# AlexanderRipar/Octree_Ray_Tracing

Measured on AMD Instinct MI355X. Metric: Mrays/sec primary traversal (depth-12 SVO-DAG, raygen+trace+shade per frame), higher is better.
Workload: dtype f32

## Files before the change

### include/och_gpu.h

```cpp
#ifndef OCH_GPU_H
#define OCH_GPU_H

#include <stddef.h>
#include <stdint.h>

#ifdef __cplusplus
extern "C" {
#endif

#define OCH_GPU_ABI_VERSION 1
#define OCH_MAX_VIEWS 8

#if defined(__GNUC__)
#define OCH_API __attribute__((visibility("default")))
#else
#define OCH_API
#endif

typedef enum och_status {
    OCH_OK = 0,
    OCH_E_INVALID = -1,
    OCH_E_HIP = -2,
    OCH_E_NODEV = -3,
    OCH_E_RCP_MODEL = -4,
// ... 17 lines not shown

typedef struct och_camera {
    float pos[3];
    float rot[9];
    float fov_factor;
    float aspect;
    float view_x;
    float view_y;
    int32_t width, height;
} och_camera;

typedef struct och_pool_info {
    uint64_t device_bytes;
    uint32_t n_nodes;
    uint32_t root;
    int32_t depth;
    int32_t index_base;
    float miss_t;
    int32_t rcp_log2_entries;
    int32_t device;
} och_pool_info;

OCH_API int och_abi_version(void);
OCH_API const char *och_last_error(void);
OCH_API int och_discarded_error(int *hip_error, int *count, char *what, size_t what_cap, int reset);
OCH_API int och_device_count(int *count);
OCH_API int och_device_list(int *devices, int capacity, int *count);

OCH_API int och_host_rcp_lut(uint32_t *lut, int *log2_entries);
OCH_API uint32_t och_rcp_from_lut(uint32_t xbits, const uint32_t *lut, int log2_entries);
OCH_API int och_rcp_lut_error(const uint32_t *lut, int log2_entries, double *max_rel_error);

OCH_API int och_gpu_pool_create(const uint32_t *nodes, uint32_t n_nodes, uint32_t root, int depth,
                                int index_base, float miss_t, int device, och_gpu_pool **out);
OCH_API int och_gpu_pool_destroy(och_gpu_pool *pool);
OCH_API int och_gpu_pool_info(const och_gpu_pool *pool, och_pool_info *info);
OCH_API int och_gpu_pool_update(och_gpu_pool *pool, uint32_t first, uint32_t count,
                                const uint32_t *nodes, uint32_t root);
OCH_API int och_gpu_set_rcp_lut(och_gpu_pool *pool, const uint32_t *lut, int log2_entries);
OCH_API int och_gpu_set_palette(och_gpu_pool *pool, const uint32_t *rgba, uint32_t n_voxels);
OCH_API int och_gpu_set_stream(och_gpu_pool *pool, void *hip_stream);
OCH_API int och_gpu_synchronize(och_gpu_pool *pool);
typedef enum och_option {
    OCH_OPT_BLOCK = 1,
    OCH_OPT_LAYOUT = 4,
    OCH_OPT_TILE_ORDER = 5,
    OCH_OPT_BOUNCE_COMPACT = 6,
    OCH_OPT_CULL = 8,
    OCH_OPT_TIMING = 10,
    OCH_OPT_PLAN = 11,
    OCH_OPT_SPLIT = 14,
    OCH_OPT_SPLIT_SEGS = 15,
    OCH_OPT_SPLIT_LEVEL = 16,
    OCH_OPT_SPLIT_TILES = 17
} och_option;
OCH_API int och_gpu_set_option(och_gpu_pool *pool, int option, int value);
OCH_API int och_gpu_get_option(const och_gpu_pool *pool, int option, int *value);
OCH_API int och_gpu_set_stamp_buffer(och_gpu_pool *pool, uint64_t *stamps, uint32_t capacity_waves);
OCH_API int och_gpu_occupancy(const och_gpu_pool *pool, int kind, int *blocks_per_cu);
OCH_API int och_gpu_last_kernel_ms(och_gpu_pool *pool, float *ms);
OCH_API int och_gpu_set_launch_events(och_gpu_pool *pool, void *start_event, void *stop_event);

OCH_API int och_gpu_trace(och_gpu_pool *pool, float ox, float oy, float oz, float dx, float dy, float dz,
                          int32_t *hit_direction, uint32_t *hit_voxel, float *hit_time);
OCH_API int och_gpu_trace_batch(och_gpu_pool *pool, const float *origin, int origin_stride,
                                const float *dirs, uint32_t n,
                                int32_t *hit_direction, uint32_t *hit_voxel, float *hit_time);
OCH_API int och_gpu_trace_batch_dev(och_gpu_pool *pool, const float *origin, int origin_stride,
                                    const float *dirs, uint32_t n,
                                    int32_t *hit_direction, uint32_t *hit_voxel, float *hit_time,
                                    uint32_t *push_count);

OCH_API int och_gpu_trace_batch_tiled_dev(och_gpu_pool *pool, const float *origin, int origin_stride,
                                          const float *dirs, uint32_t n, uint32_t width,
                                          int32_t *hit_direction, uint32_t *hit_voxel, float *hit_time,
                                          uint32_t *push_count);
OCH_API int och_gpu_trace_batch_image(och_gpu_pool *pool, const float *origin, int origin_stride,
                                      const float *dirs, uint32_t n, uint32_t width,
                                      int32_t *hit_direction, uint32_t *hit_voxel, float *hit_time);
OCH_API int och_gpu_plan_batch_tiled(och_gpu_pool *pool, const float *origin, int origin_stride,
                                     const float *dirs, uint32_t n, uint32_t width);

OCH_API int och_gpu_trace_bounce_batch_dev(och_gpu_pool *pool, const float *origin, int origin_stride,
                                           const float *dirs, uint32_t n,
                                           int32_t *hit_direction, uint32_t *hit_voxel, float *hit_time,
                                           int32_t *bounce_direction, uint32_t *bounce_voxel, float *bounce_time,
                                           uint32_t *push_count);

OCH_API int och_camera_setup(float px, float py, float pz, float yaw, float pitch, float fov,
                             int width, int height, och_camera *cam);
OCH_API int och_gpu_raygen_dev(och_gpu_pool *pool, const och_camera *cam, float *dirs);
OCH_API int och_gpu_render(och_gpu_pool *pool, const och_camera *cam, uint32_t *rgba);
OCH_API int och_gpu_render_dev(och_gpu_pool *pool, const och_camera *cam, uint32_t *rgba_slice,
                               int row_chunk, int shard, int n_shards);
OCH_API int och_shard_rows(int height, int row_chunk, int n_shards);
OCH_API int och_gpu_render_views_dev(och_gpu_pool *pool, const och_camera *cams, int n_views, uint32_t *rgba_slices,
                                     int row_chunk, int shard, int n_shards);
OCH_API int och_gpu_plan_views(och_gpu_pool *pool, const och_camera *cams, int n_views, int row_chunk, int shard,
                               int n_shards);
OCH_API int och_gpu_render_bounce_views_dev(och_gpu_pool *pool, const och_camera *cams, int n_views,
                                            uint32_t *rgba_slices, int row_chunk, int shard, int n_shards);
OCH_API int och_gpu_render_ssaa_views_dev(och_gpu_pool *pool, const och_camera *cams, int n_views, int s,
                                          uint32_t *rgba, size_t capacity_pixels);
OCH_API int och_gpu_render_ssaa(och_gpu_pool *pool, const och_camera *cam, int s, uint32_t *rgba,
                                size_t capacity_pixels);
enum { OCH_LIGHT_SUN = 1, OCH_LIGHT_AO = 2 };
typedef struct och_light {
// ... 228 lines not shown
```

### octree_ray_tracing_amd/csrc/och_internal.h

```cpp
#pragma once
#include <hip/hip_runtime.h>
#include <stdint.h>

#include <vector>

#include "../../include/och_gpu.h"
#include "och_tiles.h"

namespace och {

struct DevPool {
    const uint32_t *nodes;
    uint32_t n_slots;
    const uint32_t *lut;
    uint32_t rcp_xlo;
    uint32_t rcp_xspan;
    uint32_t root;
    int32_t packed;
    int32_t depth;
    int32_t lut_shift;
    uint32_t miss_bits;
    float half_voxel;
    uint32_t dim_lo;
    uint32_t dim_span;
    int32_t cull;
    float cull_lo[3], cull_hi[3];
    int32_t cam_cull;
};

constexpr double kCameraCullRcpError = 0x1p-10;

bool occupied_box(const uint32_t *nodes, uint32_t n_nodes, uint32_t root, int depth, int base, int32_t lo[3],
                  int32_t hi[3]);

int report(int status, const char *msg);

void clear_pending_error(const char *launcher);
struct EntryScope {
    const char *prev;
    explicit EntryScope(const char *name);
    ~EntryScope();
};
#define OCH_ENTRY() const och::EntryScope och_entry_scope_(__func__)

int pool_drain(och_gpu_pool *pool);
int pool_write_slots(och_gpu_pool *pool, uint32_t first, uint32_t count, const uint32_t *raw,
                     const uint32_t *packed, bool full);
int pool_commit(och_gpu_pool *pool, uint32_t root, uint32_t packed_root, bool packed, uint64_t writer,
                const int32_t *box_lo, const int32_t *box_hi);
int pool_mark_torn(och_gpu_pool *pool);
int pool_scatter_slots(och_gpu_pool *pool, const uint32_t *ids, uint32_t count, const uint32_t *raw,
                       const uint32_t *packed);
hipError_t launch_scatter_slots(const uint32_t *ids, const uint32_t *raw, const uint32_t *packed, uint32_t count,
                                uint32_t *d_raw, uint32_t *d_packed, hipStream_t stream);
uint64_t pool_serial(const och_gpu_pool *pool);
void *pool_stream(const och_gpu_pool *pool);
int pool_palette_size(const och_gpu_pool *pool, int *n_voxels);
uint64_t pool_last_writer(const och_gpu_pool *pool);

int comm_ranks(const och_comm *comm, int *n_ranks, int *rank, int *device);
int comm_all_gather(och_comm *comm, const void *send, void *recv, size_t bytes, hipStream_t stream);
int comm_gather(och_comm *comm, const void *send, void *recv, size_t bytes, int root, hipStream_t stream);
void comm_abort(och_comm *comm);

struct DevFrame {
    och_camera cams[OCH_MAX_VIEWS];
    int32_t n_views;
    const uint32_t *palette;
    uint32_t n_voxels;
    uint32_t *out;
    uint8_t *codes;
    int32_t row_chunk, shard, n_shards, slice_rows;
    const int32_t *chunk_map;
};

constexpr int kBounceBlock = 256;

struct Schedule {
    int block;
    int tile_order;
// ... 50 lines not shown
```

### octree_ray_tracing_amd/csrc/och_kernels.hip

```cpp
#include <hip/hip_ext.h>
#include <hip/hip_runtime.h>
#include <stdint.h>

#include <type_traits>

#include "och_internal.h"

#define OCH_LAUNCH_TIMED(sc, kernel, grid, block, lds, stream, ...)                                                   \
    do {                                                                                                             \
        clear_pending_error(__func__);                                                                               \
        if ((sc).ev_start || (sc).ev_stop)                                                                           \
            hipExtLaunchKernelGGL(kernel, grid, block, (uint32_t)(lds), stream, (sc).ev_start, (sc).ev_stop, 0u,     \
                                  __VA_ARGS__);                                                                      \
        else                                                                                                         \
            hipLaunchKernelGGL(kernel, grid, block, lds, stream, __VA_ARGS__);                                       \
    } while (0)

namespace och {
namespace {

constexpr uint32_t kX86DefaultNaN = 0xFFC00000u;

constexpr int kMaxViews = OCH_MAX_VIEWS;

// ... 492 lines not shown

struct FastDiv {
    uint32_t d, m, s;
    __host__ void init(uint32_t divisor)
    {
        d = divisor ? divisor : 1u;
        divisor = d;
        s = 0;
        while ((1ull << s) < divisor) ++s;
        m = (uint32_t)((((1ull << s) - divisor) << 32) / divisor + 1);
    }
    __device__ __forceinline__ uint32_t div(uint32_t n) const
    {
        return (uint32_t)(((uint64_t)__umulhi(n, m) + n) >> s);
    }
};

struct TiledArraySource {
    static constexpr bool kProvenMiss = false;
    static constexpr bool kTileTable = false;
    const float *origin;
    const float *dirs;
    int origin_stride;
    uint32_t n, width, tiles_x, tiles;
    FastDiv by_tiles_x;
    __host__ __device__ __forceinline__ uint32_t count() const { return tiles * 64u; }
    __device__ __forceinline__ bool at(uint32_t tile, uint32_t lane, float *o, float *d, uint32_t &out) const
    {
        const uint32_t ty = by_tiles_x.div(tile), tx = tile - ty * tiles_x;
        const uint32_t col = tx * 8u + (lane & 7u), row = ty * 8u + (lane >> 3);
        if (col >= width) return false;
        const uint32_t i = row * width + col;
        if (i >= n) return false;
        const float *po = origin + (size_t)origin_stride * i;
        const float *pd = dirs + 3 * (size_t)i;
        o[0] = po[0]; o[1] = po[1]; o[2] = po[2];
        d[0] = pd[0]; d[1] = pd[1]; d[2] = pd[2];
        out = i;
        return true;
    }
    __device__ __forceinline__ bool get_wave_culled(uint32_t wave_base, uint32_t lane, const DevPool &, bool,
                                                    float *o, float *d, uint32_t &out, bool &miss) const
    {
        miss = false;
        return at(__builtin_amdgcn_readfirstlane(wave_base >> 6), lane, o, d, out);
    }
};

struct CameraSource {
    static constexpr bool kProvenMiss = true;
    static constexpr bool kTileTable = true;
    och_camera cam[kMaxViews];
    CameraView view[kMaxViews];
    int32_t row_chunk, shard, n_shards, slice_rows, width, height;
    uint32_t slice_pixels, n_tiles;
    const uint2 *tiles;
    FastDiv by_row_chunk;
    const int32_t *chunk_map;
    __device__ __forceinline__ int global_row(int chunk, int within) const
    {
        const int g = chunk_map ? chunk_map[chunk] : chunk * n_shards + shard;
        return g < 0 ? height : g * row_chunk + within;
    }
    __host__ __device__ __forceinline__ uint32_t count() const { return n_tiles * 64u; }
    __device__ __forceinline__ bool get_wave_culled(uint32_t wave_base, uint32_t lane, const DevPool &P, bool cull,
                                                    float *o, float *d, uint32_t &out, bool &miss) const
    {
        return get_tile_culled(tile(wave_base), lane, P, cull, o, d, out, miss);
    }
    __device__ __forceinline__ bool get_tile_culled(uint2 e, uint32_t lane, const DevPool &P, bool cull, float *o, float *d,
                                                    uint32_t &out, bool &miss) const
    {
        uint32_t view;
        int col, srow, row;
        miss = false;
        if (!locate(e, lane, view, col, srow, row)) return false;
        const och_camera &C = cam[view];
        out = view * slice_pixels + (uint32_t)srow * (uint32_t)width + (uint32_t)col;
        float ru, rv, rw;
        camera_rot(C, col, row, ru, rv, rw);
        if (cull && P.cam_cull && camera_proven_miss(this->view[view], ru, rv, rw)) {
            miss = true;
            return true;
        }
        o[0] = C.pos[0]; o[1] = C.pos[1]; o[2] = C.pos[2];
        camera_ray_from(ru, rv, rw, d);
        return true;
    }
    __device__ __forceinline__ uint2 tile(uint32_t wave_base) const
    {
#if defined(__HIP_DEVICE_COMPILE__)
        typedef const __attribute__((address_space(4))) uint32_t *table_ptr;
#else
        typedef const uint32_t *table_ptr;
#endif
        const table_ptr w = (table_ptr)(uintptr_t)tiles + 2u * __builtin_amdgcn_readfirstlane(wave_base >> 6);
        const uint2 e = make_uint2(w[0], w[1]);
        return make_uint2(__builtin_amdgcn_readfirstlane(e.x), __builtin_amdgcn_readfirstlane(e.y));
    }
    __device__ __forceinline__ uint32_t sample_word(uint32_t wave_base, uint32_t lane, int log2_s) const
    {
        const uint2 e = tile(wave_base);
        const uint32_t w = (uint32_t)width >> log2_s, h = (uint32_t)height >> log2_s;
        const uint32_t x = (e.x & 0xFFFFu) + lane % kTileW, y = (e.y >> 16) + lane / kTileW;
        return (((e.x >> 16) & 15u) * h + (y >> log2_s)) * w + (x >> log2_s);
    }
    __device__ __forceinline__ bool locate(uint2 e, uint32_t lane, uint32_t &view, int &col, int &srow, int &row) const
    {
        if (e.x & kTileEmpty) return false;
        view = (e.x >> 16) & 15u;
        col = (int)((e.x & 0xFFFFu) + lane % kTileW);
        srow = (int)((e.y >> 16) + lane / kTileW);
        row = (int)((e.y & 0xFFFFu) + lane / kTileW);
        if (e.x & kTileInside) return true;
        if (col >= width || srow >= slice_rows) return false;
        if (e.x & kTileRows) {
            const int chunk = (int)by_row_chunk.div((uint32_t)srow);
            row = global_row(chunk, srow - chunk * row_chunk);
        }
        return row < height;
    }
};


template <bool kCount>
struct HitSink {
    int32_t *dir;
    uint32_t *voxel;
    uint32_t *t;
    uint32_t *push;
    __device__ __forceinline__ void put(uint32_t i, const Hit &h) const
    {
        dir[i] = h.dir;
        voxel[i] = h.voxel;
// ... 151 lines not shown
    if (key != ~0u) atomicMin(&lds_stack[best0 + pix], (key << 6) | lane);
    __syncthreads();
    if (valid) {
        const uint32_t b = lds_stack[best0 + pix];
        if (b == ~0u ? seg == 0u : (b & 63u) == lane) K.put(out, h);
    }
}

template <class Src, class Sink, int kPacked, bool kCount, bool kSplit, bool kDiag>
__global__ __attribute__((amdgpu_num_sgpr(80))) void k_trace_grid(DevPool P, Src S, Sink K, const uint32_t *__restrict__ order,
                             uint32_t *__restrict__ cost, uint64_t *stamps, uint32_t stamp_cap,
                             const uint32_t *__restrict__ split_tasks, uint32_t split_level)
{
    extern __shared__ uint32_t lds_stack[];
    if constexpr (!kDiag) {
        cost = nullptr;
        stamps = nullptr;
    }
    const uint64_t t0 = stamps ? realtime() : 0;
    const uint64_t c0 = cost ? __builtin_amdgcn_s_memtime() : 0;
    uint32_t blk = blockIdx.x;
    if constexpr (!Src::kTileTable) blk = order ? order[blockIdx.x] : blockIdx.x;
    const uint32_t lane = threadIdx.x & 63u;
    const uint32_t wave_base = kSplit ? blk * 64u : blk * blockDim.x + (threadIdx.x & ~63u);
    float o[3], d[3];
    uint32_t out;
    bool miss, have;
    if constexpr (Src::kTileTable) {
        const uint2 ent = S.tile(wave_base);
        if constexpr (kSplit) {
            if (ent.x >> 31) {
                split_tile<Src, Sink, kPacked>(P, S, K, ent, split_tasks, split_level, lds_stack);
                if (stamps) stamp(stamps, stamp_cap, t0, 64);
                return;
            }
        }
        have = S.get_tile_culled(ent, lane, P, kCount ? P.cull == 2 : P.cull != 0, o, d, out, miss);
    } else {
        have = wave_base + lane < S.count() &&
               S.get_wave_culled(wave_base, lane, P, kCount ? P.cull == 2 : P.cull != 0, o, d, out, miss);
    }
    if (have) {
        if (miss) {
            K.put(out, Hit{OCH_EXIT, 0u, P.miss_bits, 0u});
        } else {
            Ray r;
            ray_trace<kPacked, kCount, true, kAsmLoad>(r, P, o, d, stack_column(lds_stack, P.depth), blockDim.x,
                                                      !(Src::kProvenMiss && P.cam_cull));
            K.put(out, ray_result<kPacked, kAsmLoad>(r, P));
        }
    }
    if (cost && threadIdx.x == 0) cost[blk] = (uint32_t)(__builtin_amdgcn_s_memtime() - c0);
    if (stamps) stamp(stamps, stamp_cap, t0, 64);
}

template <uint32_t kBit>
__device__ __forceinline__ uint32_t lane_xor(uint32_t v)
{
    if constexpr (kBit == 1u)
        return (uint32_t)__builtin_amdgcn_update_dpp(0, (int)v, 0xB1, 0xF, 0xF, true);
    else if constexpr (kBit == 2u)
        return (uint32_t)__builtin_amdgcn_update_dpp(0, (int)v, 0x4E, 0xF, 0xF, true);
    else if constexpr (kBit == 8u)
        return (uint32_t)__builtin_amdgcn_update_dpp(0, (int)v, 0x128, 0xF, 0xF, true);
    else if constexpr (kBit == 4u || kBit == 16u)
        return (uint32_t)__builtin_amdgcn_ds_swizzle((int)v, (int)(0x1Fu | (kBit << 10)));
    else {
        static_assert(kBit == 32u, "a lane bit");
        return __builtin_amdgcn_permlane32_swap(v, v, false, false)[1];
    }
}

template <int kLog2S>
__device__ __forceinline__ uint32_t block_sum(uint32_t v)
{
    v += lane_xor<1u>(v);
    v += lane_xor<8u>(v);
    if constexpr (kLog2S >= 2) {
        v += lane_xor<2u>(v);
        v += lane_xor<16u>(v);
    }
    if constexpr (kLog2S >= 3) {
        v += lane_xor<4u>(v);
        v += lane_xor<32u>(v);
    }
    return v;
}

template <int kLog2S>
__device__ __forceinline__ void ssaa_resolve(uint32_t *out, uint32_t word, uint32_t lane, uint32_t colour)
{
    constexpr uint32_t kS = 1u << kLog2S;
    const uint32_t rb = block_sum<kLog2S>(colour & 0x00FF00FFu), ga = block_sum<kLog2S>((colour >> 8) & 0x00FF00FFu);
    if (word != ~0u && (lane & (kS - 1u)) == 0 && ((lane >> 3) & (kS - 1u)) == 0) {
        constexpr uint32_t half = (kS * kS / 2u) * 0x00010001u;
        out[word] = (((rb + half) >> (2 * kLog2S)) & 0x00FF00FFu) | ((((ga + half) >> (2 * kLog2S)) & 0x00FF00FFu) << 8);
    }
}

template <int kPacked, int kLog2S>
__global__ __attribute__((amdgpu_num_sgpr(80))) void k_trace_ssaa(DevPool P, CameraSource S, FrameSink K, uint64_t *stamps,
                                                                  uint32_t stamp_cap)
{
    extern __shared__ uint32_t lds_stack[];
    const uint64_t t0 = stamps ? realtime() : 0;
    const uint32_t blk = blockIdx.x;
// ... 450 lines not shown
                                                            int row_chunk, int n_shards, int slice_rows, int n_views,
                                                            const int32_t *__restrict__ owner, int sun_shade, int ao_shade)
{
    __shared__ uint32_t lut[256];
    lut[threadIdx.x] = table[threadIdx.x];
    __syncthreads();
    const int col = (blockIdx.x * 256 + threadIdx.x) * 4;
    const int row = blockIdx.y, view = blockIdx.z;
    if (col >= width || row >= height) return;
    const size_t src = gathered_row(row, row_chunk, n_shards, slice_rows, n_views, view, owner) * width + col;
    typedef uint32_t u32x2 __attribute__((ext_vector_type(2)));
    typedef uint32_t u32x4 __attribute__((ext_vector_type(4)));
    const u32x2 c = __builtin_nontemporal_load(reinterpret_cast<const u32x2 *>(gathered + src));
    const u32x4 px = {lit_code_word(lut, c.x & 0xFFFFu, sun_shade, ao_shade), lit_code_word(lut, c.x >> 16, sun_shade, ao_shade),
                      lit_code_word(lut, c.y & 0xFFFFu, sun_shade, ao_shade), lit_code_word(lut, c.y >> 16, sun_shade, ao_shade)};
    __builtin_nontemporal_store(px, reinterpret_cast<u32x4 *>(frames + ((size_t)view * height + row) * width + col));
}

__global__ __launch_bounds__(256) void k_scatter_slots(const uint32_t *__restrict__ ids,
                                                       const uint32_t *__restrict__ raw,
                                                       const uint32_t *__restrict__ packed, uint32_t count,
                                                       uint32_t *__restrict__ d_raw, uint32_t *__restrict__ d_packed)
{
    const uint32_t i = blockIdx.x * 256u + threadIdx.x;
    if (i >= count * 8u) return;
    const uint32_t slot = ids[i >> 3], w = i & 7u;
    d_raw[(size_t)slot * 8 + w] = raw[i];
    if (packed) d_packed[(size_t)slot * 8 + w] = packed[i];
}

constexpr size_t kStaticLds = 64;
size_t stack_bytes(int depth, int block)
{
    const size_t e = (size_t)(depth + 1) * block, c = (e + 2) / 3;
    return 4 * (c > kStaticLds ? c : kStaticLds) + 4 * e;
}

bool tiles_fit(const Schedule &sc, int block)
{
    return sc.tiles && block > 0 && sc.tiles_block == (uint32_t)block &&
           (uint64_t)sc.tiles_grid * ((uint32_t)block / 64u) <= sc.tiles_n;
}

template <class Src, class Sink, int kPacked, bool kCount>
hipError_t launch_as(const DevPool &p, const Src &s, const Sink &k, uint32_t n, const Schedule &sc, hipStream_t stream)
{
    if (!Src::kTileTable && n == 0) return hipSuccess;
    const int block = sc.block;
    const size_t lds = stack_bytes(p.depth, block);
    const uint32_t grid = (n + (uint32_t)block - 1) / (uint32_t)block;
    if constexpr (Src::kTileTable) {
        if (!tiles_fit(sc, block)) return hipErrorInvalidValue;
        const bool diag = sc.cost || sc.stamps;
        if (sc.split_tasks) {
            if constexpr (kPacked && !kCount) {
                if (block != 64) return hipErrorInvalidValue;
                if (diag)
                    OCH_LAUNCH_TIMED(sc, (k_trace_grid<Src, Sink, kPacked, kCount, true, true>), dim3(sc.tiles_grid),
                                     dim3(block), lds, stream, p, s, k, nullptr, sc.cost, sc.stamps, sc.stamp_cap,
                                     sc.split_tasks, sc.split_level);
                else
                    OCH_LAUNCH_TIMED(sc, (k_trace_grid<Src, Sink, kPacked, kCount, true, false>), dim3(sc.tiles_grid),
                                     dim3(block), lds, stream, p, s, k, nullptr, nullptr, nullptr, 0u, sc.split_tasks,
                                     sc.split_level);
                return hipGetLastError();
            }
            return hipErrorInvalidValue;
        }
        if (diag)
            OCH_LAUNCH_TIMED(sc, (k_trace_grid<Src, Sink, kPacked, kCount, false, true>), dim3(sc.tiles_grid), dim3(block),
                             lds, stream, p, s, k, nullptr, sc.cost, sc.stamps, sc.stamp_cap, nullptr, 0u);
        else
            OCH_LAUNCH_TIMED(sc, (k_trace_grid<Src, Sink, kPacked, kCount, false, false>), dim3(sc.tiles_grid), dim3(block),
                             lds, stream, p, s, k, nullptr, nullptr, nullptr, 0u, nullptr, 0u);
        return hipGetLastError();
    }
    OCH_LAUNCH_TIMED(sc, (k_trace_grid<Src, Sink, kPacked, kCount, false, true>), dim3(grid), dim3(block), lds, stream, p, s,
                     k, sc.order_n == grid ? sc.order : nullptr, sc.cost, sc.stamps, sc.stamp_cap, nullptr,
                     0u);
    return hipGetLastError();
}

template <class Src, class Sink, bool kCount>
hipError_t launch(const DevPool &p, const Src &s, const Sink &k, uint32_t n, const Schedule &sc, hipStream_t stream)
{
    return p.packed ? launch_as<Src, Sink, 1, kCount>(p, s, k, n, sc, stream)
                    : launch_as<Src, Sink, 0, kCount>(p, s, k, n, sc, stream);
}

template <class Src, class Sink, bool kCount>
hipError_t launch_bounce(const DevPool &p, const Src &s, const Sink &k, uint32_t n, const Schedule &sc, hipStream_t stream)
{
    if (!Src::kTileTable && n == 0) return hipSuccess;
    const int block = sc.block > kBounceBlock ? sc.block : kBounceBlock;
    const size_t queue = 8u * (size_t)block * sizeof(uint32_t);
    const size_t lds = stack_bytes(p.depth, block) > queue ? stack_bytes(p.depth, block) : queue;
    dim3 grid((n + block - 1) / block);
    const uint32_t *order = sc.order_n == grid.x ? sc.order : nullptr;
    if constexpr (Src::kTileTable) {
        if (!tiles_fit(sc, block) || sc.split_tasks) return hipErrorInvalidValue;
        grid.x = sc.tiles_grid;
        order = nullptr;
    }
    if (p.packed)
        OCH_LAUNCH_TIMED(sc, (k_trace_bounce<Src, Sink, 1, kCount>), grid, dim3(block), lds, stream, p, s, k,
                         sc.bounce_compact, order, sc.cost, sc.stamps, sc.stamp_cap);
    else
        OCH_LAUNCH_TIMED(sc, (k_trace_bounce<Src, Sink, 0, kCount>), grid, dim3(block), lds, stream, p, s, k,
                         sc.bounce_compact, order, sc.cost, sc.stamps, sc.stamp_cap);
    return hipGetLastError();
}

CameraSource camera_source(const DevPool &p, const DevFrame &f, const Schedule &sc)
{
    CameraSource src;
    for (int v = 0; v < f.n_views; ++v) {
        src.cam[v] = f.cams[v];
        CameraView &V = src.view[v];
        V.pos_ok = 1;
        for (int a = 0; a < 3; ++a) {
            const float o = f.cams[v].pos[a];
            const float lo = p.cull_lo[a] - 0x1p-16F, hi = p.cull_hi[a] + 0x1p-16F;
            V.lo[a] = lo - o;
            V.hi[a] = hi - o;
            V.pos_ok &= (o > 1.0F && o < 2.0F) ? 1 : 0;
        }
    }
    src.row_chunk = f.row_chunk;
    src.shard = f.shard;
    src.n_shards = f.n_shards;
    src.slice_rows = f.slice_rows;
    src.width = f.cams[0].width;
    src.height = f.cams[0].height;
    src.slice_pixels = (uint32_t)f.slice_rows * (uint32_t)src.width;
    src.by_row_chunk.init((uint32_t)src.row_chunk);
    src.tiles = reinterpret_cast<const uint2 *>(sc.tiles);
    src.n_tiles = sc.tiles ? sc.tiles_n : 0u;
    src.chunk_map = f.chunk_map;
    return src;
}

struct CameraArgs {
    CameraSource src;
    FrameSink sink;
};

bool camera_args(const DevPool &p, const DevFrame &f, const Schedule &sc, bool wave_scan, CameraArgs &c)
{
    if (f.n_views < 1 || f.n_views > kMaxViews) return false;
    if (wave_scan && (uint32_t)sc.block > 1024u) return false;
    c.src = camera_source(p, f, sc);
    c.sink = FrameSink{f.out, f.palette, f.n_voxels};
    return true;
}

bool whole_frame_samples(const DevFrame &f, int log2_s)
{
    if (f.n_shards != 1 || f.shard != 0 || f.row_chunk != f.cams[0].height || f.slice_rows != f.cams[0].height)
        return false;
    const int s = 1 << log2_s;
    return f.cams[0].width % s == 0 && f.cams[0].height % s == 0;
}

template <class Launch>
hipError_t with_layout_and_samples(const DevPool &p, int log2_s, Launch launch)
{
    const auto samples = [&](auto layout) {
        switch (log2_s) {
        case 1: return launch(layout, std::integral_constant<int, 1>{});
        case 2: return launch(layout, std::integral_constant<int, 2>{});
        case 3: return launch(layout, std::integral_constant<int, 3>{});
        default: return hipErrorInvalidValue;
        }
    };
    return p.packed ? samples(std::integral_constant<int, 1>{}) : samples(std::integral_constant<int, 0>{});
}

template <class... Params, class... Args>
hipError_t launch_tiles(const Schedule &sc, int depth, uint32_t queue_words, hipStream_t stream,
// ... 228 lines not shown
```

### octree_ray_tracing_amd/csrc/och_pool.cpp

```cpp
#include <algorithm>
#include <atomic>
#include <cstdarg>
#include <cstdio>
#include <mutex>
#include <unordered_map>

#include "och_pool.h"

using och::DeviceGuard;
using och::fail;
using och::host_rcp;
using och::HostRcp;
using och::lut_max_rel_error;

namespace {

constexpr uint32_t kIdLimit = 1u << 24;

thread_local std::string g_error;

}

int och::fail(int status, const char *fmt, ...)
{
// ... 623 lines not shown
{
    return fail(OCH_E_INVALID, "option %d was retired (the grid schedule alone remains; DESIGN.md section 8)", option);
}

}

OCH_API int och_gpu_set_option(och_gpu_pool *p, int option, int value)
{
    if (!p) return fail(OCH_E_INVALID, "pool is NULL");
    switch (option) {
    case OCH_OPT_BLOCK:
        if (value < 64 || value > 1024 || value % 64) return fail(OCH_E_INVALID, "block %d", value);
        p->opt_block = value;
        return OCH_OK;
    case OCH_OPT_LAYOUT:
        if (value != 0 && value != 1) return fail(OCH_E_INVALID, "layout must be 0 or 1");
        if (value == 1 && !p->d_packed.d) return fail(OCH_E_INVALID, "pool too large for the packed layout");
        p->opt_layout = value;
        return OCH_OK;
    case OCH_OPT_TILE_ORDER:
        if (value < 0 || value > 3) return fail(OCH_E_INVALID, "tile order must be 0..3");
        p->opt_tile_order = value;
        return OCH_OK;
    case OCH_OPT_BOUNCE_COMPACT:
        if (value < 0 || value > 2) return fail(OCH_E_INVALID, "bounce compaction must be 0, 1 or 2");
        p->opt_bounce_compact = value;
        return OCH_OK;
    case OCH_OPT_CULL:
        if (value < 0 || value > 2) return fail(OCH_E_INVALID, "cull must be 0, 1 or 2");
        p->opt_cull = value;
        return OCH_OK;
    case OCH_OPT_TIMING:
        if (value < 0 || value > 2) return fail(OCH_E_INVALID, "timing must be 0, 1 or 2");
        p->opt_timing = value;
        return OCH_OK;
    case OCH_OPT_PLAN:
        if (value < 0 || value > 100) return fail(OCH_E_INVALID, "plan shape must be 0..100");
        p->opt_plan = value;
        return OCH_OK;
    case OCH_OPT_SPLIT:
        if (value < 0 || value > 100) return fail(OCH_E_INVALID, "split threshold must be 0..100 (%% of the costliest tile)");
        p->opt_split = value;
        return OCH_OK;
    case OCH_OPT_SPLIT_SEGS:
        if (value != 2 && value != 4 && value != 8 && value != 16) return fail(OCH_E_INVALID, "split segments must be 2, 4, 8 or 16");
        p->opt_split_segs = value;
        return OCH_OK;
    case OCH_OPT_SPLIT_LEVEL:
        if (value < 1 || value > 21) return fail(OCH_E_INVALID, "split level must be 1..21");
        p->opt_split_level = value;
        return OCH_OK;
    case OCH_OPT_SPLIT_TILES:
        return fail(OCH_E_INVALID, "OCH_OPT_SPLIT_TILES is read-only");
    case 0: case 2: case 3: case 7: case 9: case 12: case 13:
        return retired_option(option);
    default:
        return fail(OCH_E_INVALID, "unknown option %d", option);
    }
}

OCH_API int och_gpu_get_option(const och_gpu_pool *p, int option, int *value)
{
    if (!p || !value) return fail(OCH_E_INVALID, "NULL argument");
    switch (option) {
    case OCH_OPT_BLOCK: *value = p->opt_block; return OCH_OK;
    case OCH_OPT_LAYOUT: *value = (p->opt_layout == 1 && p->d_packed.d) ? 1 : 0; return OCH_OK;
    case OCH_OPT_TILE_ORDER: *value = p->opt_tile_order; return OCH_OK;
    case OCH_OPT_BOUNCE_COMPACT: *value = p->opt_bounce_compact; return OCH_OK;
    case OCH_OPT_CULL: *value = p->opt_cull; return OCH_OK;
    case OCH_OPT_TIMING: *value = p->opt_timing; return OCH_OK;
    case OCH_OPT_PLAN: *value = p->opt_plan; return OCH_OK;
    case OCH_OPT_SPLIT: *value = p->opt_split; return OCH_OK;
    case OCH_OPT_SPLIT_SEGS: *value = p->opt_split_segs; return OCH_OK;
    case OCH_OPT_SPLIT_LEVEL: *value = p->opt_split_level; return OCH_OK;
    case OCH_OPT_SPLIT_TILES: *value = (int)p->split.tiles; return OCH_OK;
    case 0: case 2: case 3: case 7: case 9: case 12: case 13:
        return retired_option(option);
    default: return fail(OCH_E_INVALID, "unknown option %d", option);
    }
}

OCH_API int och_gpu_set_stamp_buffer(och_gpu_pool *p, uint64_t *stamps, uint32_t capacity_waves)
{
    if (!p) return fail(OCH_E_INVALID, "pool is NULL");
    p->stamps = capacity_waves ? stamps : nullptr;
    p->stamp_cap = stamps ? capacity_waves : 0;
    return OCH_OK;
}

OCH_API int och_gpu_set_launch_events(och_gpu_pool *p, void *start_event, void *stop_event)
{
    if (!p) return fail(OCH_E_INVALID, "pool is NULL");
    p->next_ev_start = static_cast<hipEvent_t>(start_event);
    p->next_ev_stop = static_cast<hipEvent_t>(stop_event);
    return OCH_OK;
}


OCH_API int och_pool_pack(const uint32_t *nodes, uint32_t n_nodes, uint32_t root, int depth, int index_base,
                          uint32_t *out, uint32_t out_capacity, uint32_t *out_nodes, uint32_t *out_root)
{
    if (!nodes || !out_nodes || !out_root) return fail(OCH_E_INVALID, "NULL argument");
    int st = validate_pool(nodes, n_nodes, root, depth, index_base);
    if (st != OCH_OK) return st;
    std::vector<uint32_t> packed;
    uint32_t proot = 0;
    if (!pack_pool(nodes, n_nodes, root, depth, index_base, packed, proot))
        return fail(OCH_E_CAPACITY, "more than 2^24 - 1 (node, level) pairs");
    *out_nodes = (uint32_t)(packed.size() / 8);
    *out_root = proot;
    if (out) {
        if (out_capacity < *out_nodes) return fail(OCH_E_CAPACITY, "output holds %u nodes, %u needed", out_capacity, *out_nodes);
        std::memcpy(out, packed.data(), packed.size() * 4);
    }
    return OCH_OK;
}

OCH_API int och_pool_occupied_box(const uint32_t *nodes, uint32_t n_nodes, uint32_t root, int depth, int index_base,
                                  int32_t lo[3], int32_t hi[3])
{
    if (!nodes || !lo || !hi) return fail(OCH_E_INVALID, "NULL argument");
    if (index_base != 0 && index_base != 1) return fail(OCH_E_INVALID, "index_base must be 0 or 1");
    const int st = validate_pool(nodes, n_nodes, root, depth, index_base);
    if (st != OCH_OK) return st;
    if (!och::occupied_box(nodes, n_nodes, root, depth, index_base, lo, hi))
        for (int a = 0; a < 3; ++a) lo[a] = hi[a] = 0;
    return OCH_OK;
}
// ... 178 lines not shown
```

### octree_ray_tracing_amd/csrc/och_pool.h

```cpp
#pragma once
#include <cmath>
#include <cstring>
#include <string>
#include <vector>

#include "och_host.h"

namespace och {

struct LaunchPlan {
    DevBuf<uint32_t> order;
    DevBuf<uint32_t> order_xcd;
    uint32_t blocks = 0;
    std::vector<uint32_t> h_order, h_order_xcd;
    uint64_t serial = 0;
    int64_t key[9] = {};
    void invalidate() { key[0] = -1; }
    bool matches(const int64_t k[9]) const { return order.d && std::memcmp(k, key, sizeof key) == 0; }
};

struct SplitPlan {
    DevBuf<uint32_t> order, tasks;
    std::vector<uint32_t> h_order, h_tasks;
    uint32_t n = 0, extra = 0, tiles = 0;
// ... 3 lines not shown

struct TileTable {
    DevBuf<uint64_t> d;
    uint32_t n = 0, grid = 0, block = 0;
    int64_t key[12] = {};
    uint64_t used = 0;
};

}


struct och_gpu_pool {
    int device = 0;
    och::DevBuf<uint32_t> d_nodes;
    uint32_t n_nodes = 0;
    uint32_t root = 0;
    int depth = 0;
    int index_base = 1;
    float miss_t = INFINITY;
    och::DevBuf<uint32_t> d_lut;
    int lut_log2 = 0;
    uint32_t rcp_xlo = 0, rcp_xspan = 0;
    double lut_error = INFINITY;
    och::DevBuf<uint32_t> d_palette;
    uint32_t n_voxels = 0;
    och::DevBuf<uint32_t> d_code_table;
    hipStream_t own_stream = nullptr;
    hipStream_t ext_stream = nullptr;
    bool use_ext = false;
    hipEvent_t ev_start = nullptr, ev_stop = nullptr;
    bool timed = false;
    int opt_block = 64;
    uint64_t *stamps = nullptr;
    uint32_t stamp_cap = 0;
    std::vector<uint32_t> mirror;
    och::DevBuf<uint32_t> d_packed;
    uint32_t packed_root = 0;
    uint32_t packed_nodes = 0;
    bool packed_by_slot = false;
    uint64_t serial = 0;
    uint64_t last_writer = 0;
    bool torn = false;
    uint64_t world = 0, world_generation = 0;
    uint32_t world_published = 0;
    int opt_layout = 1;
    int opt_tile_order = 0;
    int opt_bounce_compact = 1;
    int opt_cull = 1;
    int opt_timing = 1;
    int opt_plan = 10;
    int opt_split = 0;
    int opt_split_segs = 4;
    int opt_split_level = 6;
    hipEvent_t next_ev_start = nullptr;
    hipEvent_t next_ev_stop = nullptr;
    bool box_any = false;
    int32_t box_lo[3] = {0, 0, 0}, box_hi[3] = {0, 0, 0};
    och::DevBuf<char> scratch;
    uint32_t *h_stage = nullptr;
    size_t stage_words = 0;
    och::DevBuf<uint32_t> d_stage;
    och::LaunchPlan plans[3];
    och::SplitPlan split;
    uint64_t plan_serial = 0;
    och::TileTable tile_tables[8];
    uint64_t tile_clock = 0;
    int deal_h = 0, deal_chunk = 0, deal_n = 0, deal_max = 0;
    uint64_t deal_serial = 0;
    och::DevBuf<int32_t> d_chunk_map;
    std::vector<int32_t> h_chunk_map;
    och::DevBuf<int32_t> d_owner;
    std::vector<int32_t> deal_table;
    bool deal_for(int H, int rc, int n) const { return deal_n && H == deal_h && rc == deal_chunk && n == deal_n; }
    int slice_rows(int H, int rc, int n) const { return deal_for(H, rc, n) ? deal_max * rc : och_shard_rows(H, rc, n); }

    hipStream_t stream() const { return use_ext ? ext_stream : own_stream; }

    hipError_t drop_packed()
    {
        packed_nodes = 0;
        packed_by_slot = false;
        return d_packed.release();
    }

    och::Schedule schedule() const
    {
        och::Schedule sc = {};
        sc.block = opt_block;
        sc.tile_order = opt_tile_order;
        sc.bounce_compact = opt_bounce_compact;
        sc.stamps = stamps;
        sc.stamp_cap = stamp_cap;
        return sc;
    }

    och::DevPool dev() const
    {
        och::DevPool p;
        const bool pk = opt_layout == 1 && d_packed.d;
        p.nodes = pk ? d_packed.d : d_nodes.d;
        p.n_slots = 8u * (pk ? packed_nodes : n_nodes);
        p.packed = pk ? 1 : 0;
        p.lut = d_lut.d;
        p.rcp_xlo = rcp_xlo;
        p.rcp_xspan = rcp_xspan;
        p.root = pk ? packed_root : root;
        p.depth = depth;
        p.lut_shift = 23 - lut_log2;
        uint32_t mb;
        std::memcpy(&mb, &miss_t, 4);
        p.miss_bits = mb;
        p.half_voxel = std::ldexp(1.0F, -(depth + 1));
        p.dim_lo = 1u << (23 - depth);
        p.dim_span = (1u << 22) - p.dim_lo;
        p.cull = box_any ? opt_cull : 0;
        p.cam_cull = lut_error <= och::kCameraCullRcpError ? 1 : 0;
        for (int a = 0; a < 3; ++a) {
            p.cull_lo[a] = 1.0F + std::ldexp((float)box_lo[a], -depth);
            p.cull_hi[a] = 1.0F + std::ldexp((float)box_hi[a], -depth);
        }
        return p;
    }
};

namespace och {

int ensure_scratch(och_gpu_pool *p, size_t bytes);
int check_ready(const och_gpu_pool *p);

struct HostRcp {
    int status = OCH_OK;
    int log2_entries = 0;
    std::vector<uint32_t> lut;
    std::string error;
};

const HostRcp &host_rcp();
double lut_max_rel_error(const uint32_t *lut, int log2_entries);

}
```

### octree_ray_tracing_amd/tracer.py

```python
from __future__ import annotations

import ctypes as C
import enum
import math

import numpy as np

from . import _lib
from ._lib import Camera, Light, OchError, call


class Direction(enum.IntEnum):
    x_pos = 0
    y_pos = 1
    z_pos = 2
    x_neg = 3
    y_neg = 4
    z_neg = 5
    exit = 6
    inside = 7
    error = 8


def _np_ptr(a: np.ndarray) -> int:
# ... 88 lines not shown
        pool.depth, pool.index_base, pool.miss_t = int(depth), int(index_base), float(miss_t)
        pool._h = handle
        pool._palette_n = 0
        return pool

    def close(self):
        if getattr(self, "_h", None) and self._h.value:
            call("och_gpu_pool_destroy", self._h)
            self._h = C.c_void_p()

    def __del__(self):
        try:
            self.close()
        except Exception:
            pass

    def __enter__(self):
        return self

    def __exit__(self, *exc):
        self.close()

    def info(self) -> dict:
        inf = _lib.PoolInfo()
        call("och_gpu_pool_info", self._h, C.byref(inf))
        return {f: getattr(inf, f) for f, _ in _lib.PoolInfo._fields_}

    def get_root(self) -> int:
        return self.info()["root"]

    def set_rcp_lut(self, lut: np.ndarray):
        lut = np.ascontiguousarray(lut, np.uint32).reshape(-1)
        if lut.size < 2 or lut.size & (lut.size - 1):
            raise ValueError("RCPPS table size must be a power of two")
        call("och_gpu_set_rcp_lut", self._h, _np_ptr(lut), int(round(math.log2(lut.size))))

    def set_palette(self, rgba: np.ndarray):
        rgba = np.ascontiguousarray(rgba, np.uint32).reshape(-1)
        if rgba.size % 6:
            raise ValueError("palette must hold 6 colours per voxel id")
        call("och_gpu_set_palette", self._h, _np_ptr(rgba), rgba.size // 6)
        self._palette_n = rgba.size // 6

    def set_stream(self, stream):
        handle = getattr(stream, "cuda_stream", stream)
        call("och_gpu_set_stream", self._h, C.c_void_p(handle))

    def update(self, first: int, nodes: np.ndarray, root: int):
        nodes = np.ascontiguousarray(nodes, np.uint32).reshape(-1, 8)
        call("och_gpu_pool_update", self._h, int(first), nodes.shape[0], _np_ptr(nodes), int(root))

    OPTIONS = {"block": 1, "layout": 4, "tile_order": 5, "bounce_compact": 6, "cull": 8, "timing": 10, "plan": 11,
               "split": 14, "split_segs": 15, "split_level": 16}
    READ_ONLY = {"split_tiles": 17}

    def set_option(self, name: str, value: int):
        call("och_gpu_set_option", self._h, self.OPTIONS[name], int(value))

    def get_option(self, name: str) -> int:
        v = C.c_int()
        call("och_gpu_get_option", self._h, self.OPTIONS.get(name) or self.READ_ONLY[name], C.byref(v))
        return v.value

    def set_stamp_buffer(self, stamps, capacity_waves: int):
        call("och_gpu_set_stamp_buffer", self._h, None if stamps is None else _dev_ptr(stamps), int(capacity_waves))

    def occupancy(self, kind: int = 0) -> int:
        v = C.c_int()
        call("och_gpu_occupancy", self._h, int(kind), C.byref(v))
        return v.value

    def synchronize(self):
        call("och_gpu_synchronize", self._h)

    def last_kernel_ms(self) -> float:
        ms = C.c_float()
        call("och_gpu_last_kernel_ms", self._h, C.byref(ms))
        return ms.value

    def set_launch_events(self, start, stop):
        call("och_gpu_set_launch_events", self._h, _event_handle(start), _event_handle(stop))

    def sse_trace(self, ox, oy, oz, dx, dy, dz):
        d, v, t = C.c_int32(), C.c_uint32(), C.c_float()
        call("och_gpu_trace", self._h, float(ox), float(oy), float(oz), float(dx), float(dy), float(dz),
             C.byref(d), C.byref(v), C.byref(t))
        return Direction(d.value), v.value, t.value

    def trace_batch(self, origins, dirs, width: int | None = None):
        dirs = np.ascontiguousarray(dirs, np.float32).reshape(-1, 3)
        origins = np.ascontiguousarray(origins, np.float32)
        stride = 0 if origins.size == 3 else 3
        n = dirs.shape[0]
        hd, hv, ht = np.empty(n, np.int32), np.empty(n, np.uint32), np.empty(n, np.float32)
        if width:
            call("och_gpu_trace_batch_image", self._h, _np_ptr(origins), stride, _np_ptr(dirs), n, int(width),
                 _np_ptr(hd), _np_ptr(hv), _np_ptr(ht))
        else:
            call("och_gpu_trace_batch", self._h, _np_ptr(origins), stride, _np_ptr(dirs), n,
                 _np_ptr(hd), _np_ptr(hv), _np_ptr(ht))
        return hd, hv, ht

    def trace_batch_dev(self, origins, dirs, hit_dir, hit_voxel, hit_time, push=None, n=None):
        if n is None:
            n = dirs.numel() // 3
        stride = 0 if origins.numel() == 3 else 3
        self._need_batch(origins, dirs, n, stride, (hit_dir, hit_voxel, hit_time, push))
        call("och_gpu_trace_batch_dev", self._h, _dev_ptr(origins), stride, _dev_ptr(dirs), int(n),
             _dev_ptr(hit_dir), _dev_ptr(hit_voxel), _dev_ptr(hit_time),
             None if push is None else _dev_ptr(push))

    def trace_batch_tiled_dev(self, origins, dirs, width: int, hit_dir, hit_voxel, hit_time, push=None, n=None):
        if n is None:
            n = dirs.numel() // 3
# ... 294 lines not shown
```

Before: 46780.

## Classify camera tiles as sky or ground to skip per-ray miss tests

Adds a per-view tile classifier built on the host: conservative fixed-point linear planes over pixel coordinates that mark whole tiles as certain sky (rays miss the occupied box) or certain ground. Sky tiles return a miss straight away, without camera rotation or traversal, and ground tiles skip the per-ray proven-miss test. The goal is to cut per-lane work on rays that leave the scene bounds. It adds plane evaluation per lane and is only correct if the error margins in the quantisation hold, so an optional verification kernel and a failure counter are included.

```diff
diff --git a/include/och_gpu.h b/include/och_gpu.h
--- a/include/och_gpu.h
+++ b/include/och_gpu.h
@@ -93,7 +93,9 @@
     OCH_OPT_SPLIT = 14,
     OCH_OPT_SPLIT_SEGS = 15,
     OCH_OPT_SPLIT_LEVEL = 16,
-    OCH_OPT_SPLIT_TILES = 17
+    OCH_OPT_SPLIT_TILES = 17,
+    OCH_OPT_TILE_CLASS = 18,
+    OCH_OPT_TILE_CLASS_FAILS = 19
 } och_option;
 OCH_API int och_gpu_set_option(och_gpu_pool *pool, int option, int value);
 OCH_API int och_gpu_get_option(const och_gpu_pool *pool, int option, int *value);
diff --git a/octree_ray_tracing_amd/csrc/och_internal.h b/octree_ray_tracing_amd/csrc/och_internal.h
--- a/octree_ray_tracing_amd/csrc/och_internal.h
+++ b/octree_ray_tracing_amd/csrc/och_internal.h
@@ -5,6 +5,7 @@
 #include <vector>
 
 #include "../../include/och_gpu.h"
+#include "och_tile_class.h"
 #include "och_tiles.h"
 
 namespace och {
@@ -26,6 +27,8 @@
     int32_t cull;
     float cull_lo[3], cull_hi[3];
     int32_t cam_cull;
+    int32_t tile_class;
+    uint32_t *class_fails;
 };
 
 constexpr double kCameraCullRcpError = 0x1p-10;
diff --git a/octree_ray_tracing_amd/csrc/och_kernels.hip b/octree_ray_tracing_amd/csrc/och_kernels.hip
--- a/octree_ray_tracing_amd/csrc/och_kernels.hip
+++ b/octree_ray_tracing_amd/csrc/och_kernels.hip
@@ -568,6 +568,7 @@
     static constexpr bool kTileTable = true;
     och_camera cam[kMaxViews];
     CameraView view[kMaxViews];
+    TileClassView cls[kMaxViews];
     int32_t row_chunk, shard, n_shards, slice_rows, width, height;
     uint32_t slice_pixels, n_tiles;
     const uint2 *tiles;
@@ -584,6 +585,11 @@
     {
         return get_tile_culled(tile(wave_base), lane, P, cull, o, d, out, miss);
     }
+    __device__ __forceinline__ int classed(uint2 e, bool cull) const
+    {
+        if (!cull || (e.x & (kTileInside | kTileRows | kTileSplit | kTileEmpty)) != kTileInside) return kClassUnknown;
+        return tile_class(cls[(e.x >> 16) & 15u], (int32_t)(e.x & 0xFFFFu), (int32_t)(e.y & 0xFFFFu));
+    }
     __device__ __forceinline__ bool get_tile_culled(uint2 e, uint32_t lane, const DevPool &P, bool cull, float *o, float *d,
                                                     uint32_t &out, bool &miss) const
     {
@@ -591,11 +597,17 @@
         int col, srow, row;
         miss = false;
         if (!locate(e, lane, view, col, srow, row)) return false;
+        out = view * slice_pixels + (uint32_t)srow * (uint32_t)width + (uint32_t)col;
+        cull = cull && P.cam_cull;
+        const int cls_of = classed(e, cull);
+        if (cls_of == kClassSky) {
+            miss = true;
+            return true;
+        }
         const och_camera &C = cam[view];
-        out = view * slice_pixels + (uint32_t)srow * (uint32_t)width + (uint32_t)col;
         float ru, rv, rw;
         camera_rot(C, col, row, ru, rv, rw);
-        if (cull && P.cam_cull && camera_proven_miss(this->view[view], ru, rv, rw)) {
+        if (cull && cls_of != kClassGround && camera_proven_miss(this->view[view], ru, rv, rw)) {
             miss = true;
             return true;
         }
@@ -853,6 +865,19 @@
     }
     if (cost && threadIdx.x == 0) cost[blk] = (uint32_t)(__builtin_amdgcn_s_memtime() - c0);
     if (stamps) stamp(stamps, stamp_cap, t0, 64);
+}
+
+__global__ void k_class_verify(DevPool P, CameraSource S, bool cull)
+{
+    const uint32_t lane = threadIdx.x & 63u;
+    const uint2 e = S.tile(blockIdx.x * blockDim.x + (threadIdx.x & ~63u));
+    uint32_t view;
+    int col, srow, row;
+    if ((e.x >> 31) || !S.locate(e, lane, view, col, srow, row)) return;
+    if (S.classed(e, cull && P.cam_cull) != kClassSky) return;
+    float ru, rv, rw;
+    camera_rot(S.cam[view], col, row, ru, rv, rw);
+    if (!camera_proven_miss(S.view[view], ru, rv, rw)) atomicAdd(P.class_fails, 1u);
 }
 
 template <uint32_t kBit>
@@ -1409,6 +1434,15 @@
     if constexpr (Src::kTileTable) {
         if (!tiles_fit(sc, block)) return hipErrorInvalidValue;
         const bool diag = sc.cost || sc.stamps;
+        if constexpr (std::is_same<Src, CameraSource>::value) {
+            if (diag && p.tile_class == 2 && p.class_fails) {
+                clear_pending_error(__func__);
+                hipLaunchKernelGGL(k_class_verify, dim3(sc.tiles_grid), dim3(block), 0, stream, p, s,
+                                   kCount ? p.cull == 2 : p.cull != 0);
+                const hipError_t e = hipGetLastError();
+                if (e != hipSuccess) return e;
+            }
+        }
         if (sc.split_tasks) {
             if constexpr (kPacked && !kCount) {
                 if (block != 64) return hipErrorInvalidValue;
@@ -1482,6 +1516,7 @@
             V.hi[a] = hi - o;
             V.pos_ok &= (o > 1.0F && o < 2.0F) ? 1 : 0;
         }
+        src.cls[v] = tile_class_view(f.cams[v], p.cull_lo, p.cull_hi, p.cull != 0 && p.cam_cull != 0, p.tile_class);
     }
     src.row_chunk = f.row_chunk;
     src.shard = f.shard;
diff --git a/octree_ray_tracing_amd/csrc/och_pool.cpp b/octree_ray_tracing_amd/csrc/och_pool.cpp
--- a/octree_ray_tracing_amd/csrc/och_pool.cpp
+++ b/octree_ray_tracing_amd/csrc/och_pool.cpp
@@ -699,6 +699,19 @@
         return OCH_OK;
     case OCH_OPT_SPLIT_TILES:
         return fail(OCH_E_INVALID, "OCH_OPT_SPLIT_TILES is read-only");
+    case OCH_OPT_TILE_CLASS:
+        if (value < 0 || value > 3) return fail(OCH_E_INVALID, "tile class must be 0..3");
+        if (value == 2) {
+            DeviceGuard g(p->device);
+            if (!g.ok) return fail(OCH_E_HIP, "hipSetDevice(%d) failed", p->device);
+            hipError_t e = p->d_class_fails.reserve(1);
+            if (e == hipSuccess) e = hipMemsetAsync(p->d_class_fails.d, 0, sizeof(uint32_t), p->stream());
+            if (e != hipSuccess) return fail(OCH_E_HIP, "tile class counter: %s", hipGetErrorString(e));
+        }
+        p->opt_tile_class = value;
+        return OCH_OK;
+    case OCH_OPT_TILE_CLASS_FAILS:
+        return fail(OCH_E_INVALID, "OCH_OPT_TILE_CLASS_FAILS is read-only");
     case 0: case 2: case 3: case 7: case 9: case 12: case 13:
         return retired_option(option);
     default:
@@ -721,6 +734,19 @@
     case OCH_OPT_SPLIT_SEGS: *value = p->opt_split_segs; return OCH_OK;
     case OCH_OPT_SPLIT_LEVEL: *value = p->opt_split_level; return OCH_OK;
     case OCH_OPT_SPLIT_TILES: *value = (int)p->split.tiles; return OCH_OK;
+    case OCH_OPT_TILE_CLASS: *value = p->opt_tile_class; return OCH_OK;
+    case OCH_OPT_TILE_CLASS_FAILS: {
+        *value = 0;
+        if (!p->d_class_fails.d) return OCH_OK;
+        DeviceGuard g(p->device);
+        if (!g.ok) return fail(OCH_E_HIP, "hipSetDevice(%d) failed", p->device);
+        uint32_t n = 0;
+        hipError_t e = hipStreamSynchronize(p->stream());
+        if (e == hipSuccess) e = hipMemcpy(&n, p->d_class_fails.d, sizeof n, hipMemcpyDeviceToHost);
+        if (e != hipSuccess) return fail(OCH_E_HIP, "tile class counter: %s", hipGetErrorString(e));
+        *value = (int)(n > 0x7FFFFFFFu ? 0x7FFFFFFFu : n);
+        return OCH_OK;
+    }
     case 0: case 2: case 3: case 7: case 9: case 12: case 13:
         return retired_option(option);
     default: return fail(OCH_E_INVALID, "unknown option %d", option);
diff --git a/octree_ray_tracing_amd/csrc/och_pool.h b/octree_ray_tracing_amd/csrc/och_pool.h
--- a/octree_ray_tracing_amd/csrc/och_pool.h
+++ b/octree_ray_tracing_amd/csrc/och_pool.h
@@ -79,6 +79,8 @@
     int opt_split = 0;
     int opt_split_segs = 4;
     int opt_split_level = 6;
+    int opt_tile_class = 1;
+    och::DevBuf<uint32_t> d_class_fails;
     hipEvent_t next_ev_start = nullptr;
     hipEvent_t next_ev_stop = nullptr;
     bool box_any = false;
@@ -142,6 +144,8 @@
         p.dim_span = (1u << 22) - p.dim_lo;
         p.cull = box_any ? opt_cull : 0;
         p.cam_cull = lut_error <= och::kCameraCullRcpError ? 1 : 0;
+        p.tile_class = opt_tile_class == 2 && !d_class_fails.d ? 1 : opt_tile_class;
+        p.class_fails = d_class_fails.d;
         for (int a = 0; a < 3; ++a) {
             p.cull_lo[a] = 1.0F + std::ldexp((float)box_lo[a], -depth);
             p.cull_hi[a] = 1.0F + std::ldexp((float)box_hi[a], -depth);
diff --git a/octree_ray_tracing_amd/csrc/och_tile_class.h b/octree_ray_tracing_amd/csrc/och_tile_class.h
--- /dev/null
+++ b/octree_ray_tracing_amd/csrc/och_tile_class.h
@@ -0,0 +1,151 @@
+#pragma once
+#include <math.h>
+#include <stdint.h>
+
+#include "../../include/och_gpu.h"
+
+#if defined(__HIPCC__) || defined(__CUDACC__)
+#define OCH_CLASS_FN __host__ __device__ __forceinline__
+#else
+#define OCH_CLASS_FN inline
+#endif
+
+namespace och {
+
+constexpr int kClassSkyPlanes = 5;
+constexpr int kClassUnknown = 0, kClassSky = 1, kClassGround = 2;
+constexpr int kClassLo = -1, kClassHi = 8;
+constexpr int kClassMaxExtent = 65535;
+
+struct TileClassView {
+    int32_t sky[kClassSkyPlanes][2];
+    int32_t band[3][3];
+    int32_t ground[2];
+    int32_t pad[3];
+};
+
+OCH_CLASS_FN int32_t class_plane(const int32_t *p, int32_t col, int32_t row)
+{
+    const int32_t a = (int32_t)(int16_t)(uint16_t)((uint32_t)p[0] & 0xFFFFu), b = p[0] >> 16;
+    return (int32_t)((uint32_t)a * (uint32_t)col + (uint32_t)b * (uint32_t)row + (uint32_t)p[1]);
+}
+
+OCH_CLASS_FN int tile_class(const TileClassView &V, int32_t col, int32_t row)
+{
+    bool sky = false;
+    for (int k = 0; k < kClassSkyPlanes; ++k) sky |= class_plane(V.sky[k], col, row) > 0;
+    if (sky) {
+        bool band = false;
+        for (int a = 0; a < 3; ++a) band |= (uint32_t)class_plane(V.band[a], col, row) <= (uint32_t)V.band[a][2];
+        if (!band) return kClassSky;
+    }
+    return class_plane(V.ground, col, row) > 0 ? kClassGround : kClassUnknown;
+}
+
+
+struct ClassForm {
+    double p, q, r;
+};
+
+inline void class_never(int32_t *plane) { plane[0] = 0, plane[1] = -1; }
+inline int32_t class_pack(double a, double b)
+{
+    return (int32_t)(((uint32_t)(int32_t)b << 16) | ((uint32_t)(int32_t)a & 0xFFFFu));
+}
+
+inline void class_quantise(const ClassForm &f, int32_t *plane)
+{
+    const double c = f.r + (f.p < 0 ? kClassHi : kClassLo) * f.p + (f.q < 0 ? kClassHi : kClassLo) * f.q;
+    const double span = 65536.0 * (fabs(f.p) + fabs(f.q)) + fabs(c);
+    if (!(span > 0x1p-200 && span < 0x1p200)) return class_never(plane);
+    const double s = 0x1p30 / span;
+    plane[0] = class_pack(floor(s * f.p), floor(s * f.q));
+    plane[1] = (int32_t)floor(s * c) - 1;
+}
+
+inline void class_band(const ClassForm &f, double w, int32_t *band)
+{
+    const double lo = fmin(kClassLo * f.p, kClassHi * f.p) + fmin(kClassLo * f.q, kClassHi * f.q);
+    const double hi = fmax(kClassLo * f.p, kClassHi * f.p) + fmax(kClassLo * f.q, kClassHi * f.q);
+    const double span = 65536.0 * (fabs(f.p) + fabs(f.q)) + fabs(f.r) + 2.0 * w + (hi - lo);
+    if (!(span > 0x1p-200 && span < 0x1p200)) {
+        band[0] = band[1] = 0, band[2] = -1;
+        return;
+    }
+    const double s = 0x1p29 / span;
+    const double q = 2.0 * kClassMaxExtent + 2.0;
+    const double first = floor(s * (-w - hi) - q) - 1.0, last = ceil(s * (w - lo)) + 1.0;
+    band[0] = class_pack(floor(s * f.p), floor(s * f.q));
+    band[1] = (int32_t)(floor(s * f.r) - first);
+    band[2] = (int32_t)(last - first);
+}
+
+inline TileClassView tile_class_view(const och_camera &C, const float *cull_lo, const float *cull_hi, bool usable,
+                                     int mode)
+{
+    TileClassView V = {};
+    for (int k = 0; k < kClassSkyPlanes; ++k) class_never(V.sky[k]);
+    for (int a = 0; a < 3; ++a) V.band[a][0] = V.band[a][1] = 0, V.band[a][2] = -1;
+    class_never(V.ground);
+    if (!usable || mode == 0) return V;
+    if (mode == 3) {
+        V.ground[1] = 1;
+        return V;
+    }
+    bool pos_ok = true;
+    for (int a = 0; a < 3; ++a) pos_ok &= C.pos[a] > 1.0F && C.pos[a] < 2.0F;
+    if (!pos_ok || C.width <= 0 || C.height <= 0) return V;
+    const double au = (double)C.aspect * (double)C.view_x, av = (double)C.view_y, f = C.fov_factor;
+    const double umax = fabs((double)C.aspect) * (fabs((double)C.view_x) * C.width + 1.0);
+    const double vmax = fabs((double)C.view_y) * C.height + 1.0;
+    const int rows[3] = {6, 0, 3};
+    const double sign[3] = {1.0, 1.0, -1.0};
+    ClassForm D[3];
+    double E[3];
+    for (int a = 0; a < 3; ++a) {
+        const double k0 = C.rot[rows[a]], k1 = C.rot[rows[a] + 1], k2 = C.rot[rows[a] + 2];
+        D[a] = ClassForm{sign[a] * au * k0, sign[a] * av * k1, sign[a] * (f * k2 - (double)C.aspect * k0 - k1)};
+        E[a] = 0x1p-20 * (umax * fabs(k0) + vmax * fabs(k1) + fabs(f * k2));
+        if (!(E[a] < 0x1p60)) return V;
+    }
+    const double emax = fmax(fmax(E[0], E[1]), E[2]), emin = fmin(fmin(E[0], E[1]), E[2]);
+    if (!(emax > 0x1p-40 && emin >= 0x1p-30 * emax)) return V;
+    double lo[3], hi[3];
+    for (int a = 0; a < 3; ++a) {
+        lo[a] = ((double)cull_lo[a] - 0x1p-15) - (double)C.pos[a];
+        hi[a] = ((double)cull_hi[a] + 0x1p-15) - (double)C.pos[a];
+    }
+    double sz, g;
+    if (hi[2] < 0.0)
+        sz = 1.0, g = -hi[2];
+    else if (lo[2] > 0.0)
+        sz = -1.0, g = lo[2];
+    else
+        return V;
+    for (int a = 0; a < 3; ++a) class_band(D[a], 2.0 * E[a], V.band[a]);
+    const auto plane = [&](double alpha, double beta, double gamma, double extra, int32_t *out) {
+        const double thr = fabs(alpha) * E[0] + fabs(beta) * E[1] + fabs(gamma) * E[2] + extra;
+        class_quantise(ClassForm{alpha * D[0].p + beta * D[1].p + gamma * D[2].p,
+                                 alpha * D[0].q + beta * D[1].q + gamma * D[2].q,
+                                 alpha * D[0].r + beta * D[1].r + gamma * D[2].r - thr},
+                       out);
+    };
+    plane(0.0, 0.0, sz, 2.0 * E[2], V.sky[0]);
+    const double m = 1.0 + 0x1p-6;
+    plane(g, 0.0, fmax(hi[0], 0.0) * m * sz, 0.0, V.sky[1]);
+    plane(-g, 0.0, fmax(-lo[0], 0.0) * m * sz, 0.0, V.sky[2]);
+    plane(0.0, g, fmax(hi[1], 0.0) * m * sz, 0.0, V.sky[3]);
+    plane(0.0, -g, fmax(-lo[1], 0.0) * m * sz, 0.0, V.sky[4]);
+    if (lo[0] < 0.0 && hi[0] > 0.0 && lo[1] < 0.0 && hi[1] > 0.0) {
+        const double cx = 0.5 * (C.width - 1), cy = 0.5 * (C.height - 1);
+        const double fx = D[0].p * cx + D[0].q * cy + D[0].r, fy = D[1].p * cx + D[1].q * cy + D[1].r;
+        const double k = 1.0 - 0x1p-6;
+        if (fabs(fx) >= fabs(fy))
+            fx >= 0.0 ? plane(-g, 0.0, -hi[0] * k * sz, 0.0, V.ground) : plane(g, 0.0, lo[0] * k * sz, 0.0, V.ground);
+        else
+            fy >= 0.0 ? plane(0.0, -g, -hi[1] * k * sz, 0.0, V.ground) : plane(0.0, g, lo[1] * k * sz, 0.0, V.ground);
+    }
+    return V;
+}
+
+}
diff --git a/octree_ray_tracing_amd/tracer.py b/octree_ray_tracing_amd/tracer.py
--- a/octree_ray_tracing_amd/tracer.py
+++ b/octree_ray_tracing_amd/tracer.py
@@ -164,14 +164,16 @@
 
     OPTIONS = {"block": 1, "layout": 4, "tile_order": 5, "bounce_compact": 6, "cull": 8, "timing": 10, "plan": 11,
                "split": 14, "split_segs": 15, "split_level": 16}
-    READ_ONLY = {"split_tiles": 17}
+    READ_ONLY = {"split_tiles": 17, "tile_class_fails": 19}
+    CLASS_OPTIONS = {"tile_class": 18}
 
     def set_option(self, name: str, value: int):
-        call("och_gpu_set_option", self._h, self.OPTIONS[name], int(value))
+        call("och_gpu_set_option", self._h, {**self.OPTIONS, **self.CLASS_OPTIONS}[name], int(value))
 
     def get_option(self, name: str) -> int:
         v = C.c_int()
-        call("och_gpu_get_option", self._h, self.OPTIONS.get(name) or self.READ_ONLY[name], C.byref(v))
+        ids = {**self.OPTIONS, **self.CLASS_OPTIONS, **self.READ_ONLY}
+        call("och_gpu_get_option", self._h, ids[name], C.byref(v))
         return v.value
 
     def set_stamp_buffer(self, stamps, capacity_waves: int):
```

Result: no change. 46910, median of 6 (+0.3%).
